# torchmd/torchmd-net

Hardware: AMD Instinct MI355X
Metric: molecules/sec (64-atom molecules) TensorNet E+F (higher is better)
Workload: dtype f32; 1 GPU; BASELINE configs[1]: TensorNet F=128 L=2 K=32 rc=5.0, S-mol64 256 molecules x 64 atoms per GPU, energies + forces, random-init weights (seed 0); atoms_per_gpu=16384, pairs_per_gpu=193709, directed_edges_per_gpu=403802, parallelism=molecule-sharded x1, RCCL all-reduce of energies, rank_step=eager: tmdnet_build_graph (pair-count read-back) + tmdnet_energy_forces

## Files before the change

include/tmdnet_amd.h:

```cpp
#ifndef TMDNET_AMD_H
#define TMDNET_AMD_H

#include <stddef.h>
#include <stdint.h>

#ifdef __cplusplus
extern "C" {
#endif

#define TMDNET_OK 0
#define TMDNET_ERR_INVALID 1
#define TMDNET_ERR_HIP 2
#define TMDNET_ERR_OVERFLOW 3
#define TMDNET_ERR_WORKSPACE 4
#define TMDNET_ERR_STATE 5

typedef struct tmdnet_model tmdnet_model;

typedef struct tmdnet_hparams {
  int32_t hidden_channels;
  int32_t num_layers;
  int32_t num_rbf;
  int32_t max_z;
  int32_t max_num_neighbors;
// ... 127 lines not shown
#define TMDNET_GEMM_ROUTE_SB1_128 6
#define TMDNET_GEMM_ROUTE_SB1_64 7
typedef struct tmdnet_gemm_ex_args {
  const float* A;
  const float* W[TMDNET_GEMM_MAX_GROUPS];
  const float* bias[TMDNET_GEMM_MAX_GROUPS];
  float* C;
  float* pre;
  const float* aux;
  const float* rowscale;
  int64_t lda, ldw, ldc, ldpre, ldaux;
  int32_t a_off[TMDNET_GEMM_MAX_GROUPS], c_off[TMDNET_GEMM_MAX_GROUPS], pre_off[TMDNET_GEMM_MAX_GROUPS],
      aux_off[TMDNET_GEMM_MAX_GROUPS];
  int32_t M, N, K, groups, flags;
  const int32_t* m_dev;
  int32_t m_add;
  const uint16_t* Wsbg[TMDNET_GEMM_MAX_GROUPS];
} tmdnet_gemm_ex_args;
int tmdnet_debug_gemm_ex(void* stream, const tmdnet_gemm_ex_args* args, int32_t* route_out);
int tmdnet_debug_tlin9(void* stream, int32_t pro, int32_t epi, int64_t N, int64_t F, const float* A, const float* A2, float* C,
                       const float* e0, const float* e1, const float* e2, const float* e3, const float* e4, float* o1, float* o2,
                       const float* kap, int32_t want_feat, const float* W_I, const float* W_A, const float* W_S,
                       uint16_t* scratch, int64_t* scratch_elems);
#define TMDNET_MSG_OP_FWD 0
#define TMDNET_MSG_OP_ADJ 1
#define TMDNET_MSG_OP_GD 2
#define TMDNET_MSG_OP_DUAL 3
#define TMDNET_MSG_AUTO 0
#define TMDNET_MSG_FWD_ROW 1
#define TMDNET_MSG_FWD_SPLIT 2
#define TMDNET_MSG_FWD_TILE 3
#define TMDNET_MSG_ADJ_ROW 4
#define TMDNET_MSG_ADJ_SPLIT 5
#define TMDNET_MSG_GD_ROW 6
#define TMDNET_MSG_GD_SPLIT 7
#define TMDNET_MSG_GD_TILE 8
#define TMDNET_MSG_DUAL 9
#define TMDNET_MSG_DUAL_ACC 10
#define TMDNET_MSG_DUAL_SPLIT3 16
typedef struct tmdnet_message_args {
  int32_t op, kernel;
  int32_t N, F, P, small_mols, o3, balance, accumulate;
  const int32_t* rowptr;
  const int32_t* col;
  const int32_t* epair;
  const float* esign;
// ... 136 lines not shown
```

torchmd-net_amd/csrc/tn_api.hip:

```cpp
#include <hip/hip_runtime.h>

#include <algorithm>
#include <cmath>
#include <cstdio>
#include <cstdlib>
#include <cstring>
#include <map>
#include <unordered_map>
#include <string>
#include <vector>

#include "tn_chain.h"
#include "tn_heads.h"
#include "tn_model.h"
#include "tn_tlin9.h"
#include "tn_small.h"
#include "tn_interp.h"
#include "tn_virial.h"

using namespace tn;

static const char* kCatNames[CAT_COUNT] = {"graph", "gemm_edge", "gemm_node", "message", "pair_bwd", "embed_scatter", "elementwise", "edge_table"};

int fail(tmdnet_model* m, int code, const std::string& msg) {
// ... 174 lines not shown
void recall_graph(tmdnet_model* m, const void* graph_ws) {
  auto it = m->graph_rec.find(graph_ws);
  if (it == m->graph_rec.end()) return;
  m->graph_is_cell = it->second.is_cell;
  m->graph_cell_multi = it->second.cell_multi;
  m->graph_has_z = it->second.has_z;
  m->last_nt = it->second.nt;
  m->lastE = it->second.lastE;
  m->graph_no_ghost_pairs = it->second.no_ghost_pairs;
}

bool tlin9_images(const float* const W3[3]) {
  if (!g_cur) return false;
  for (int t = 0; t < 3; ++t)
    if (g_cur->fm_of.find(W3[t]) == g_cur->fm_of.end()) return false;
  return true;
}
void tlin9(hipStream_t s, int pro, int epi, const float* const W3[3], Tl9Args a, double tensors, const char* what) {
  for (int t = 0; t < 3; ++t) a.Wfm[t] = g_cur->fm_of.at(W3[t]);
  char lab[64];
  std::snprintf(lab, sizeof(lab), "tlin9 %s 9x%dx%dx%d", what, a.N, a.F, a.F);
  ProfScope ps_(s, CAT_GEMM_NODE, 2.0 * 9 * a.N * (double)a.F * a.F, 4.0 * (tensors * 9.0 * a.N * a.F + 3.0 * a.F * a.F), lab);
  launch_tlin9(a, pro, epi, s);
}

Graph carve_graph(void* ws, int64_t N, int64_t B, int64_t ecap, size_t* total) {
  Carver c(ws);
  Graph g{};
  const int64_t pcap = ecap / 2 + 1;
  g.small_mols = N <= 96 * (B > 0 ? B : 1) ? 1 : 0;
  g.counts = c.take<int>(8);
  g.mstart = c.take<int>(B);
  g.mend = c.take<int>(B);
  g.nlow = c.take<int>(N);
  g.ntot = c.take<int>(N);
  g.rowptr = c.take<int>(N + 1);
  g.pairptr = c.take<int>(N + 1);
  g.col = c.take<int>(ecap);
  g.epair = c.take<int>(ecap);
  g.esign = c.take<float>(ecap);
  g.pair_i = c.take<int>(pcap);
  g.pair_j = c.take<int>(pcap);
  g.pd = c.take<float>(pcap + 1);
  g.pdelta = c.take<float>(pcap * 3);
  g.prhat = c.take<float>(pcap * 3);
  g.ecap = ecap;
// ... 842 lines not shown
  HIP_TRY(m, hipGetLastError());
  return TMDNET_OK;
}

int tmdnet_set_option(tmdnet_model* m, const char* name, double value) {
  if (!m || !name) return TMDNET_ERR_INVALID;
  const std::string n(name);
  if (n == "edge_table_min_pairs") {
    m->tab_min_pairs = value < 0 ? 0 : (int64_t)value;
    return TMDNET_OK;
  }
  if (n == "embed_rb_min_atoms") {
    m->rb_min_atoms = value < 0 ? 0 : (int64_t)value;
    return TMDNET_OK;
  }
  if (n == "chain_min_atoms") {
    m->chain_min_atoms = value < 0 ? 0 : (value > 9e18 ? INT64_MAX : (int64_t)value);
    return TMDNET_OK;
  }
  if (n == "chain_mask") {
    m->chain_mask = (int)value & 7;
    return TMDNET_OK;
  }
  if (n == "pair_rows_bf16") {
    if (!m->et) return fail(m, TMDNET_ERR_INVALID, "pair_rows_bf16 applies to the Equivariant Transformer handle only");
    m->pair_bf16 = value == 2.0 ? 2 : (value != 0.0 ? 1 : 0);
    return TMDNET_OK;
  }
  if (n == "recompute_pair_rows") {
    if (m->et || m->tn2) return fail(m, TMDNET_ERR_INVALID, "recompute_pair_rows applies to the TensorNet handle only");
    m->recompute_rows = value != 0.0;
    return TMDNET_OK;
  }
  return fail(m, TMDNET_ERR_INVALID, "unknown option: " + n);
}

int tmdnet_get_info(const tmdnet_model* m, const char* name, double* value) {
  if (!m || !name || !value) return TMDNET_ERR_INVALID;
  const std::string n(name);
  if (m->tabs_pending && n.rfind("edge_table_", 0) == 0 && n != "edge_table_min_pairs")
    if (const int rc = ensure_radial_tables(const_cast<tmdnet_model*>(m), nullptr)) return rc;
  if (n == "edge_table_T") *value = m->tabs.ok ? m->tabs.T : 0;
  else if (n == "edge_table_err_value") *value = m->tabs.err_value;
  else if (n == "edge_table_err_slope") *value = m->tabs.err_slope;
  else if (n == "edge_table_min_pairs") *value = (double)m->tab_min_pairs;
  else if (n == "pair_rows_bf16") *value = (double)m->pair_bf16;
  else if (n == "embed_rb_min_atoms") *value = (double)m->rb_min_atoms;
  else if (n == "chain_min_atoms") *value = (double)m->chain_min_atoms;
  else if (n == "chain_mask") *value = (double)m->chain_mask;
  else if (n == "chain_last") *value = (double)m->chain_last;
  else if (n == "recompute_pair_rows") *value = m->recompute_rows ? 1.0 : 0.0;
  else if (n == "embed_rb") *value = m->rb_fwd ? 1.0 : 0.0;
  else if (n == "species_last_build") *value = (double)m->last_nt;
  else if (n == "halo_active_first") *value = (double)m->halo_active[0];
  else if (n == "halo_active_rows") *value = (double)m->halo_active[1];
  else if (n == "message_route_last") *value = (double)m->msg_route_last[0];
  else if (n == "message_adjoint_route_last") *value = (double)m->msg_route_last[1];
  else return TMDNET_ERR_INVALID;
  return TMDNET_OK;
}

int tmdnet_set_cell_grid(tmdnet_model* m, int32_t ncx, int32_t ncy, int32_t ncz) {
  if (!m) return TMDNET_ERR_INVALID;
  if (ncx < 0 || ncy < 0 || ncz < 0) ncx = ncy = ncz = -1;
  m->cell_n[0] = ncx;
  m->cell_n[1] = ncy;
  m->cell_n[2] = ncz;
  return TMDNET_OK;
}

int tmdnet_graph_workspace_bytes(const tmdnet_model* m, int64_t n_atoms, int64_t n_mol, size_t* bytes) {
  if (!m || !bytes || n_atoms < 0 || n_mol < 0) return TMDNET_ERR_INVALID;
  const int64_t ecap = (int64_t)m->hp.max_num_neighbors * n_atoms;
// ... 286 lines not shown
  }
  const bool use_mid = !small_fused_ok(N, F, H, L);
  auto HALO = [&](int stage, float* rows, int row_floats) -> int {
    if (!m->halo_fn) return 0;
    return m->halo_fn(m->halo_user, stage, rows, (int64_t)N, (int64_t)row_floats, perm, (void*)s);
  };
#define HALO_TRY(stage, rows, row_floats) \
  do { if (HALO(stage, rows, row_floats)) return fail(m, TMDNET_ERR_STATE, "halo exchange callback failed at stage " + std::to_string(stage)); } while (0)
  int a0 = 0, Na = N;
  if (m->halo_fn && m->halo_rng && m->atom_w && m->graph_is_cell && want_forces && !tc && (int64_t)N > 256 * (int64_t)B) {
    int h[4] = {0, 0, 0, 0};
    launch_owned_range(m->atom_w, perm, N, m->halo_rng, s);
    HIP_TRY(m, hipMemcpyAsync(h, m->halo_rng, sizeof(h), hipMemcpyDeviceToHost, s));
    HIP_TRY(m, hipStreamSynchronize(s));
    const bool images = tlin9_images(W.Ue) && tlin9_images(W.UeT) && L > 0 && tlin9_images(W.layer[0].V) && tlin9_images(W.layer[0].VT);
    if (h[2] > 0 && h[2] < N && h[1] - h[0] + 1 == h[2] && images && tlin9_ok(h[2], F, true)) {
      a0 = h[0];
      Na = h[2];
    }
  }
  const bool rng = Na != N;
  const bool t9 = !tc && tlin9_ok(Na, F, rng) && tlin9_images(W.Ue) && tlin9_images(W.UeT) && (L == 0 || tlin9_images(W.layer[0].V));
  const bool t9r = !tc && L > 0 && tlin9_ok(Na, F, rng) && tlin9_images(W.UeT) && tlin9_images(W.layer[0].VT);
  m->halo_active[0] = a0;
  m->halo_active[1] = Na;
  const int64_t o1_ = a0, oF = (int64_t)a0 * F, o2F = 2 * oF, o3F = 3 * oF, o9F = 9 * oF, oH = (int64_t)a0 * H;
  const float* const q_a = q ? q + o1_ : nullptr;
  const int64_t* const batch_a = batch_k ? batch_k + o1_ : nullptr;
  const bool fused_small = !tc && !ntp && !recompute && !m->halo_fn && !m->head_kind && (small_fused_ok(N, F, H, L) || mid_fused_ok(N, F, H, L)) &&
                           (!want_forces || (message_adjoint_gd_ok(N, F) && !getenv("TMDNET_SEPARATE_PAIR_GD")));
  auto fm_image = [&](const float* w) -> const uint16_t* {
    auto it = m->fm_of.find(w);
    return it == m->fm_of.end() ? nullptr : it->second;
  };
  const bool chain_any = !tc && !m->head_kind && !m->halo_fn && Na == N && !fused_small && (int64_t)N >= m->chain_min_atoms;
  const bool chain_ro = chain_any && (m->chain_mask & 1) && want_forces && run_fwd && run_bwd && chain_readout_shape_ok(F, H) &&
                        fm_image(W.Lin) && fm_image(W.LinT) && fm_image(W.O1) && fm_image(W.O1T);
  const bool chain_gate = chain_any && want_forces && run_fwd && run_bwd && chain_gate_shape_ok(F);
  const bool chain_gf = chain_gate && (m->chain_mask & 2) && fm_image(W.L1) && fm_image(W.L2);
  const bool chain_gb = chain_gate && (m->chain_mask & 4) && fm_image(W.L2T) && fm_image(W.L1T);
  m->chain_last = (chain_ro ? 1 : 0) | (chain_gf ? 2 : 0) | (chain_gb ? 4 : 0);
  if (run_fwd) {
    if (use_tab) {
      const float* tabs[8];
      float* outs[8];
      float* douts[8];
      int nt_ = 0;
      if (!ntp) {
        tabs[nt_] = m->tabs.tab[0];
        outs[nt_] = b.Q;
        douts[nt_++] = want_forces ? b.dQ : nullptr;
// ... 81 lines not shown
      KR(CAT_SCATTER, momB + Nd * 10 * Fd * 4, launch_embed_combine(g, N, F, K, ntp, z, W.Utab, W.Vtab, m->rb_fwd, b.mom, b.u0, b.s0n, s));
    } else {
      KR(CAT_SCATTER, Pd * 12 * Fd + E_ * 12 + Nd * 10 * Fd * 4,
         launch_embed_scatter(g, N, F, z, W.Utab, W.Vtab, b.Q, b.C, b.u0, b.s0n, s));
    }
    NODE();
    if (chain_gf) {
      ChainGateFwdArgs ca{};
      ca.s0n = b.s0n; ca.xh0 = b.xh0; ca.rstd0 = b.rstd0; ca.a1 = b.a1; ca.a2 = b.a2; ca.gates = b.gates;
      ca.ln_w = W.ln0_w; ca.ln_b = W.ln0_b; ca.bL1 = W.bL1; ca.bL2 = W.bL2; ca.L1_fm = fm_image(W.L1); ca.L2_fm = fm_image(W.L2); ca.N = N;
      char lab[64];
      std::snprintf(lab, sizeof(lab), "chain gate_fwd %dx%d", N, F);
      ProfScope ps_(s, CAT_GEMM_NODE, 2.0 * Nd * 8.0 * Fd * Fd, Nd * 10 * Fd * 4 + Nd * 4 + 4.0 * 8.0 * Fd * Fd, lab);
      if (launch_chain_gate_fwd(ca, F, s)) return fail(m, TMDNET_ERR_HIP, "launch_chain_gate_fwd");
    } else {
    KR(CAT_ELEMENTWISE, Nd * Fd * 12,
       launch_layernorm_fwd(b.s0n + oF, W.ln0_w, W.ln0_b, Na, F, b.ln0 + oF, b.xh0 + oF, b.rstd0 + o1_, s));
    gemm(s, b.ln0 + oF, F, W.L1, F, W.bL1, b.h1 + o2F, 2 * F, Na, 2 * F, F, GEMM_ACT_SILU, b.a1 + o2F, 2 * F);
    gemm(s, b.h1 + o2F, 2 * F, W.L2, 2 * F, W.bL2, b.gates + o3F, 3 * F, Na, 3 * F, 2 * F, GEMM_ACT_SILU, b.a2 + o3F, 3 * F);
    }
    if (t9) {
      Tl9Args ta{};
      ta.A = b.u0 + o9F; ta.C = b.X[0] + o9F; ta.o1 = b.UX + o9F; ta.e3 = b.gates + o3F; ta.N = Na; ta.F = F;
      tlin9(s, TL9_PRO_PLAIN, TL9_EPI_MULGATE, W.Ue, ta, 3.0 + 1.0 / 3.0, "gate");
    } else
      tensor_linear(s, b.u0, W.Ue, b.X[0], N, F, GEMM_MUL_AUX, b.UX, b.gates);
    for (int l = 0; l < L; ++l) {
      const LayerP& q_ = W.layer[l];
      if (es != s) HIP_TRY(m, hipStreamWaitEvent(s, m->ev_join[l], 0));
      float* const Xh_l = tc ? tc->Xh[l] : b.Xh;
      float* const Ch_l = tc ? tc->Ch[l] : b.Ch;
      float* const Xh_n = tc && l + 1 < L ? tc->Xh[l + 1] : b.Xh;
      if (t9) {
        Tl9Args ta{};
        ta.A = b.X[l] + o9F; ta.C = b.Pn[l] + o9F; ta.N = Na; ta.F = F;
        tlin9(s, TL9_PRO_NORM, TL9_EPI_PLAIN, q_.V, ta, 2.0, "norm");
        HALO_TRY(l, b.Pn[l], 9 * F);
        m->msg_route_last[0] = message_route(g, N, F, recompute, a0, rng ? Na : -1);
        KR(CAT_MESSAGE, wB + idxB + nodeB * (1.0 + 2.0 * Na / Nd),
           launch_message(g, N, F, b.w[l], b.Pn[l], q, batch_k, o3, b.Mi[l], Ch_l, s, recompute ? &rts[l] : nullptr, a0, rng ? Na : -1));
        Tl9Args tb{};
        tb.A = Ch_l + o9F; tb.C = b.D[l] + o9F; tb.e0 = b.X[l] + o9F; tb.o1 = b.X[l + 1] + o9F; tb.o2 = b.feat + o3F;
        tb.want_feat = l + 1 == L; tb.kap = q_a;
        tb.N = Na; tb.F = F;
        tlin9(s, TL9_PRO_PLAIN, TL9_EPI_UPDATE, q_.V + 3, tb, 4.0 + (l + 1 == L ? 1.0 / 3.0 : 0.0), "update");
        continue;
      }
      if (l == 0) KR(CAT_ELEMENTWISE, 2 * nodeB, launch_norm_x(b.X[l], Xh_l, N, F, s));
      tensor_linear(s, Xh_l, q_.V, b.Pn[l], N, F);
      HALO_TRY(l, b.Pn[l], 9 * F);
      m->msg_route_last[0] = message_route(g, N, F, recompute);
      KR(CAT_MESSAGE, wB + idxB + 3 * nodeB, launch_message(g, N, F, b.w[l], b.Pn[l], q, batch_k, o3, b.Mi[l], Ch_l, s, recompute ? &rts[l] : nullptr));
      tensor_linear(s, Ch_l, q_.V + 3, b.D[l], N, F);
      KR(CAT_ELEMENTWISE, 4 * nodeB, launch_layer_update(Xh_l, b.D[l], q, batch_k, N, F, b.X[l + 1], l + 1 < L ? 1 : 2,
                                                         l + 1 < L ? Xh_n : b.feat, s));
    }
    if (L == 0) KR(CAT_ELEMENTWISE, nodeB + Nd * 3 * Fd * 4, launch_readout_feat(b.X[L] + o9F, Na, F, b.feat + o3F, s));
    if (chain_ro) {
      ChainReadoutArgs ca{};
      ca.feat = b.feat; ca.X = b.X[L]; ca.G = b.G; ca.x = b.x; ca.ea = b.ea;
      ca.lnr_w = W.lnr_w; ca.lnr_b = W.lnr_b; ca.bLin = W.bLin; ca.bO1 = W.bO1; ca.O2 = W.O2; ca.bO2 = W.bO2;
      ca.Lin_fm = fm_image(W.Lin); ca.LinT_fm = fm_image(W.LinT); ca.O1_fm = fm_image(W.O1); ca.O1T_fm = fm_image(W.O1T);
      ca.atomref = W.atomref; ca.z = z; ca.aw = m->atom_w; ca.perm = perm; ca.std_ = W.std; ca.N = N;
      {
        char lab[64];
        std::snprintf(lab, sizeof(lab), "chain readout_fb %dx%dx%d", N, F, H);
        ProfScope ps_(s, CAT_GEMM_NODE, 2.0 * Nd * (2.0 * 3 * Fd * Fd + 2.0 * Fd * H),
                      2 * nodeB + Nd * 4 * Fd * 4 + Nd * 4 + 4.0 * (2.0 * 3 * Fd * Fd + 2.0 * Fd * H), lab);
// ... 604 lines not shown
  Tl9Args a{};
  for (int t = 0; t < 3; ++t) {
    launch_split_weight_fm(W3[t], F, F, scratch + t * one, s);
    a.Wfm[t] = scratch + t * one;
  }
  a.A = A;
  a.A2 = A2;
  a.C = C;
  a.e0 = e0;
  a.e1 = e1;
  a.e2 = e2;
  a.e3 = e3;
  a.e4 = e4;
  a.o1 = o1;
  a.o2 = o2;
  a.kap = kap;
  a.N = (int)N;
  a.F = (int)F;
  a.want_feat = want_feat ? 1 : 0;
  if (hipGetLastError() != hipSuccess) return TMDNET_ERR_HIP;
  return launch_tlin9(a, pro, epi, s) == (int)hipSuccess ? TMDNET_OK : TMDNET_ERR_HIP;
}

static_assert(TMDNET_MSG_FWD_ROW == MSG_FWD_ROW && TMDNET_MSG_FWD_SPLIT == MSG_FWD_SPLIT && TMDNET_MSG_FWD_TILE == MSG_FWD_TILE &&
                  TMDNET_MSG_ADJ_ROW == MSG_ADJ_ROW && TMDNET_MSG_ADJ_SPLIT == MSG_ADJ_SPLIT && TMDNET_MSG_GD_ROW == MSG_GD_ROW &&
                  TMDNET_MSG_GD_SPLIT == MSG_GD_SPLIT && TMDNET_MSG_GD_TILE == MSG_GD_TILE && TMDNET_MSG_DUAL == MSG_DUAL &&
                  TMDNET_MSG_DUAL_ACC == MSG_DUAL_ACC && TMDNET_MSG_DUAL_SPLIT3 == MSG_DUAL_SPLIT3 && TMDNET_MSG_AUTO == MSG_NONE,
              "route values of the header");

int tmdnet_debug_message(void* stream, const tmdnet_message_args* x, int32_t* route_out, int32_t* slot_arrays_out) {
  if (!x) return TMDNET_ERR_INVALID;
  const int N = x->N, F = x->F;
  if (N < 1 || F < 1 || x->P < 0 || x->op < TMDNET_MSG_OP_FWD || x->op > TMDNET_MSG_OP_DUAL) return TMDNET_ERR_INVALID;
  if (!x->rowptr || !x->col || !x->epair || !x->esign || !x->counts) return TMDNET_ERR_INVALID;
  Graph g{};
  g.rowptr = const_cast<int*>(x->rowptr);
  g.col = const_cast<int*>(x->col);
  g.epair = const_cast<int*>(x->epair);
  g.esign = const_cast<float*>(x->esign);
  g.counts = const_cast<int*>(x->counts);
  g.small_mols = x->small_mols ? 1 : 0;
  MsgRoute r = static_cast<MsgRoute>(x->kernel);
  const bool automatic = x->kernel == TMDNET_MSG_AUTO;
  if (automatic) {
    switch (x->op) {
      case TMDNET_MSG_OP_FWD: r = message_route(g, N, F); break;
// ... 57 lines not shown
```

torchmd-net_amd/csrc/tn_model.h:

```cpp
#pragma once
#include <hip/hip_runtime.h>

#include <cstdio>
#include <cstring>
#include <map>
#include <string>
#include <unordered_map>
#include <vector>

#include "../../include/tmdnet_amd.h"
#include "tn_gemm.h"
#include "tn_kernels.h"
#include "tn_train.h"

using namespace tn;


struct LayerP {
  const float *M1, *b1, *M2, *b2, *M3, *b3;
  const float *M2T, *M3T;
  const float* V[6];
  const float* VT[6];
  const uint16_t* M_sb[3];
};
// ... 151 lines not shown
  std::vector<ParamSpec> specs;
  std::map<std::string, std::vector<float>> host;
  float* dev = nullptr;
  size_t dev_cap = 0, dev_sb_cap = 0, rb_cap = 0;
  uint16_t* dev_sb = nullptr;
  std::unordered_map<const float*, const uint16_t*> sb_of;
  std::unordered_map<const float*, const uint16_t*> fm_of;
  struct ImageJob { size_t src_off; int64_t n, k; size_t dst_off; int fm; };
  std::vector<ImageJob> image_jobs;
  size_t packed_elems = 0;
  int32_t* upd_tid = nullptr;
  int32_t* upd_ofs = nullptr;
  const float** upd_ptrs = nullptr;
  bool upd_ready = false;
  DevParams P;
  EdgeTables tabs;
  uint16_t* rb_img = nullptr;
  const uint16_t *rb_fwd = nullptr, *rb_rev = nullptr;
  int last_nt = 0;
  int64_t rb_min_atoms = 1024;
  int64_t chain_min_atoms = 4096;
  int chain_mask = 7;
  int chain_last = 0;
  int pair_bf16 = 0;
  bool tabs_pending = false;
  int64_t tab_min_pairs = 1;
  bool finalized = false;
  std::string err;
  FwdBuffers last{};
  int64_t lastN = 0, lastP = 0;
  bool has_last = false;
  const float* tn2_last_chg = nullptr;
};


int fail(tmdnet_model* m, int code, const std::string& msg);
#define HIP_TRY(m, expr)                                                                    \
  do {                                                                                      \
    hipError_t e_ = (expr);                                                                 \
    if (e_ != hipSuccess) return fail(m, TMDNET_ERR_HIP, std::string(#expr) + ": " + hipGetErrorString(e_)); \
  } while (0)

struct Packer {
  std::vector<float> buf;
  size_t add(const std::vector<float>& v) {
    size_t off = (buf.size() + 63) & ~size_t(63);
// ... 86 lines not shown
```

torchmd-net_amd/csrc/tn_tlin9.h:

```cpp
#pragma once
#include <hip/hip_runtime.h>
#include <stdint.h>

namespace tn {

enum Tl9Pro : int {
  TL9_PRO_PLAIN = 0,
  TL9_PRO_NORM,
  TL9_PRO_UPDBWD,
};
enum Tl9Epi : int {
  TL9_EPI_PLAIN = 0,
  TL9_EPI_MULGATE,
  TL9_EPI_UPDATE,
  TL9_EPI_NORMBWD,
  TL9_EPI_NORMBWD_GATE,
  TL9_EPI_EMBBWD,
};

struct Tl9Args {
  const float* A;
  const float* A2;
  const uint16_t* Wfm[3];
  float* C;
  const float* e0;
  const float* e1;
  const float* e2;
  const float* e3;
  const float* e4;
  float* o1;
  float* o2;
  const float* kap;
  int N, F, o3, want_feat;
};

bool tlin9_ok(int N, int F, bool any_rounds = false);
size_t split_weight_fm_elems(int64_t n, int64_t k);
void launch_split_weight_fm(const float* W_dev, int64_t n, int64_t k, uint16_t* out_dev, hipStream_t s);
int launch_tlin9(const Tl9Args& a, int pro, int epi, hipStream_t s);

}
```

torchmd-net_amd/csrc/tn_tlin9.hip:

```cpp
#include <cstdlib>

#include "tn_common.h"
#include "tn_gemm_sb.h"
#include "tn_tlin9.h"

namespace tn {

constexpr int T9_RA = 32;
constexpr int T9_PLANE = 9 * T9_RA * 32;
constexpr int T9_STAGE = 3 * T9_PLANE;
constexpr int T9_EG = 8;
constexpr int T9_NT = 128;

typedef float f2v __attribute__((ext_vector_type(2)));
__device__ __forceinline__ f2v ld2(const float* p) { return *reinterpret_cast<const f2v*>(p); }
__device__ __forceinline__ void st2(float* p, f2v v) { *reinterpret_cast<f2v*>(p) = v; }
__device__ __forceinline__ f2v ldu2(const float* ubase, unsigned off) {
  return *reinterpret_cast<const f2v*>(reinterpret_cast<const char*>(ubase) + (size_t)(off * 4u));
}
__device__ __forceinline__ float ldu1(const float* ubase, unsigned off) {
  return *reinterpret_cast<const float*>(reinterpret_cast<const char*>(ubase) + (size_t)(off * 4u));
}
__device__ __forceinline__ void stu2(float* ubase, unsigned off, f2v v) {
  *reinterpret_cast<f2v*>(reinterpret_cast<char*>(ubase) + (size_t)(off * 4u)) = v;
// ... 13 lines not shown
__device__ __forceinline__ void t9_update(const float x[9], const float d[9], float kap, float o[9]) {
  float xh[9];
#pragma unroll
  for (int c = 0; c < 9; ++c) xh[c] = x[c];
  t9_norm(xh);
  const M3 dX = compose(d);
  const M3 Xf = add(add(compose(xh), dX), scale(matmul(dX, dX), kap));
  decompose(Xf, o);
}
__device__ __forceinline__ void t9_norm_bwd(const float u[9], float gx[9] ) {
  float dq[9];
  dquad(u, dq);
  const float inv = 1.0f / (quad(u) + 1.0f);
  float dot = 0.f;
#pragma unroll
  for (int c = 0; c < 9; ++c) dot += gx[c] * u[c];
  const float g_s = -dot * inv * inv;
#pragma unroll
  for (int c = 0; c < 9; ++c) gx[c] = gx[c] * inv + dq[c] * g_s;
}

template <int N_> struct IC { static constexpr int value = N_; };

template <int PRO, int EPI>
__global__ __launch_bounds__(512, 2) void k_tlin9(Tl9Args a, int tiles_m, int tiles_n) {
  __shared__ __attribute__((aligned(16))) unsigned char sA[4 * T9_STAGE];
  float* const sE = reinterpret_cast<float*>(sA + 2 * T9_STAGE);
  const int tid = threadIdx.x, lane = tid & 63, wave = tid >> 6;
  const int wave_u = __builtin_amdgcn_readfirstlane(wave);
  const int wn = wave & 3, wc = wave >> 2;
  const int sa = tid >> 4, skp = tid & 15;
  const int N = a.N, F = a.F, nd = F >> 5, NB = F >> 5;
  const int F9 = 9 * F;
  const int total = tiles_m * tiles_n;
  if ((int)blockIdx.x >= total) return;
  const int my_tiles = (total - 1 - (int)blockIdx.x) / (int)gridDim.x + 1;
  const int ndt = my_tiles * nd;

  auto tile_of = [&](int ts, int& m0, int& n0) __attribute__((always_inline)) {
    const int t = (int)blockIdx.x + ts * (int)gridDim.x;
    const int tn_ = t % tiles_n;
    m0 = (t / tiles_n) * T9_RA;
    n0 = tn_ * T9_NT;
  };

  f2v sr[2][9];
  f2v sr2[2][9];
  float s_kap[2];
  auto load_dbl = [&](auto S_, int dd) __attribute__((always_inline)) {
    constexpr int S = decltype(S_)::value;
    dd = dd < ndt ? dd : ndt - 1;
    const int ts = dd / nd, kd = dd - ts * nd;
    int m0, n0;
    tile_of(ts, m0, n0);
    int n = m0 + sa;
    if (n >= N) n = N - 1;
    if (PRO == TL9_PRO_UPDBWD) s_kap[S] = a.kap ? a.kap[n] : 1.0f;
    const unsigned voff = (unsigned)((n - m0) * F9 + skp * 2);
    const float* p = a.A + (int64_t)m0 * F9 + kd * 32;
#pragma unroll
    for (int c = 0; c < 9; ++c) sr[S][c] = ldu2(p + c * F, voff);
    if (PRO == TL9_PRO_UPDBWD) {
      const float* p2 = a.A2 + (int64_t)m0 * F9 + kd * 32;
// ... 289 lines not shown
    for (int ts = 0; ts < my_tiles; ++ts) {
      int m0n = m0c, n0n = n0c;
      if (ts + 1 < my_tiles) tile_of(ts + 1, m0n, n0n);
#pragma unroll
      for (int ci = 0; ci < 5; ++ci)
#pragma unroll
        for (int e = 0; e < 16; ++e) acc[ci][e] = 0.f;
      for (int kd = 0; kd < nd; kd += 2) {
        dbl(IC<0>{}, ROT_, kd, n0n);
        dbl(IC<1>{}, ROT_, kd + 1, n0n);
      }
      epi_group(IC<0>{}, m0c, n0c);
      epi_group(IC<1>{}, m0c, n0c);
      epi_group(IC<2>{}, m0c, n0c);
      epi_group(IC<3>{}, m0c, n0c);
      m0c = m0n;
      n0c = n0n;
    }
  };
  if (wave < 4) run(IC<0>{});
  else run(IC<1>{});
}

__global__ void k_split_weight_fm(const float* __restrict__ W, int n, int k, uint16_t* __restrict__ out) {
  const int idx = blockIdx.x * blockDim.x + threadIdx.x;
  const int NB = n >> 5, nkc = k >> 4;
  if (idx >= nkc * NB * 64) return;
  const int lane = idx & 63, nb = (idx >> 6) % NB, kc = (idx >> 6) / NB;
  const float* src = W + (int64_t)(nb * 32 + (lane & 31)) * k + kc * 16 + 8 * (lane >> 5);
  const float4 u = *reinterpret_cast<const float4*>(src), v = *reinterpret_cast<const float4*>(src + 4);
  uint4 h, m, l;
  split8(u, v, h, m, l);
  uint16_t* o = out + (((int64_t)kc * NB + nb) * 3) * 512 + lane * 8;
  *reinterpret_cast<uint4*>(o) = h;
  *reinterpret_cast<uint4*>(o + 512) = m;
  *reinterpret_cast<uint4*>(o + 1024) = l;
}
size_t split_weight_fm_elems(int64_t n, int64_t k) { return (size_t)(n * k * 3); }
void launch_split_weight_fm(const float* W_dev, int64_t n, int64_t k, uint16_t* out_dev, hipStream_t s) {
  const int total = (int)((k >> 4) * (n >> 5) * 64);
  hipLaunchKernelGGL(k_split_weight_fm, dim3((total + 255) / 256), dim3(256), 0, s, W_dev, (int)n, (int)k, out_dev);
}

static int t9_num_cu() {
  static const int n_cu = [] {
    int dev = 0, n = 256;
// ... 12 lines not shown
  const int64_t n_cu = t9_num_cu(), rounds = (tiles + n_cu - 1) / n_cu;
  return tiles <= n_cu || 5 * tiles >= 4 * rounds * n_cu;
}

int launch_tlin9(const Tl9Args& a, int pro, int epi, hipStream_t s) {
  const int tiles_m = (a.N + T9_RA - 1) / T9_RA, tiles_n = a.F / T9_NT;
  const int n_cu = t9_num_cu();
  const int total = tiles_m * tiles_n;
  const dim3 grid(total < n_cu ? total : n_cu), block(512);
#define T9_LAUNCH(P, E) hipLaunchKernelGGL((k_tlin9<P, E>), grid, block, 0, s, a, tiles_m, tiles_n)
  if (pro == TL9_PRO_NORM && epi == TL9_EPI_PLAIN) T9_LAUNCH(TL9_PRO_NORM, TL9_EPI_PLAIN);
  else if (pro == TL9_PRO_PLAIN && epi == TL9_EPI_PLAIN) T9_LAUNCH(TL9_PRO_PLAIN, TL9_EPI_PLAIN);
  else if (pro == TL9_PRO_PLAIN && epi == TL9_EPI_MULGATE) T9_LAUNCH(TL9_PRO_PLAIN, TL9_EPI_MULGATE);
  else if (pro == TL9_PRO_PLAIN && epi == TL9_EPI_UPDATE) T9_LAUNCH(TL9_PRO_PLAIN, TL9_EPI_UPDATE);
  else if (pro == TL9_PRO_UPDBWD && epi == TL9_EPI_PLAIN) T9_LAUNCH(TL9_PRO_UPDBWD, TL9_EPI_PLAIN);
  else if (pro == TL9_PRO_PLAIN && epi == TL9_EPI_NORMBWD) T9_LAUNCH(TL9_PRO_PLAIN, TL9_EPI_NORMBWD);
  else if (pro == TL9_PRO_PLAIN && epi == TL9_EPI_NORMBWD_GATE) T9_LAUNCH(TL9_PRO_PLAIN, TL9_EPI_NORMBWD_GATE);
  else if (pro == TL9_PRO_PLAIN && epi == TL9_EPI_EMBBWD) T9_LAUNCH(TL9_PRO_PLAIN, TL9_EPI_EMBBWD);
  else return (int)hipErrorInvalidValue;
#undef T9_LAUNCH
  return (int)hipGetLastError();
}

}
```

torchmd-net_amd/torchmdnet_amd/_C.py:

```python
import ctypes as C
import os
import re

_HERE = os.path.dirname(os.path.abspath(__file__))
LIB_PATH = os.path.join(os.path.dirname(_HERE), "lib", "libtmdnet_amd.so")
HEADER_PATH = os.path.join(os.path.dirname(os.path.dirname(_HERE)), "include", "tmdnet_amd.h")

OK, ERR_INVALID, ERR_HIP, ERR_OVERFLOW, ERR_WORKSPACE, ERR_STATE = 0, 1, 2, 3, 4, 5
HEAD_SCALAR, HEAD_DIPOLE_MOMENT, HEAD_SPATIAL_EXTENT, HEAD_VECTOR = 0, 1, 2, 3


class HParams(C.Structure):
    _fields_ = [
        ("hidden_channels", C.c_int32),
        ("num_layers", C.c_int32),
        ("num_rbf", C.c_int32),
        ("max_z", C.c_int32),
        ("max_num_neighbors", C.c_int32),
        ("group_o3", C.c_int32),
        ("head_hidden", C.c_int32),
        ("has_atomref", C.c_int32),
        ("cutoff_lower", C.c_float),
        ("cutoff_upper", C.c_float),
    ]
# ... 10 lines not shown
                                         "head_hidden", "has_atomref", "q_dim")] + \
               [("cutoff_lower", C.c_float), ("cutoff_upper", C.c_float), ("coulomb_cutoff", C.c_float),
                ("coulomb_epsilon_solvent", C.c_float)]


class GemmExArgs(C.Structure):
    _fields_ = [
        ("A", C.c_void_p), ("W", C.c_void_p * 9), ("bias", C.c_void_p * 9), ("C", C.c_void_p), ("pre", C.c_void_p),
        ("aux", C.c_void_p), ("rowscale", C.c_void_p),
        ("lda", C.c_int64), ("ldw", C.c_int64), ("ldc", C.c_int64), ("ldpre", C.c_int64), ("ldaux", C.c_int64),
        ("a_off", C.c_int32 * 9), ("c_off", C.c_int32 * 9), ("pre_off", C.c_int32 * 9), ("aux_off", C.c_int32 * 9),
        ("M", C.c_int32), ("N", C.c_int32), ("K", C.c_int32), ("groups", C.c_int32), ("flags", C.c_int32),
        ("m_dev", C.c_void_p), ("m_add", C.c_int32),
        ("Wsbg", C.c_void_p * 9),
    ]


class MessageArgs(C.Structure):
    _fields_ = [(n, C.c_int32) for n in ("op", "kernel", "N", "F", "P", "small_mols", "o3", "balance", "accumulate")] + \
               [(n, C.c_void_p) for n in ("rowptr", "col", "epair", "esign", "counts", "w", "w2", "src", "src2", "q", "batch", "out",
                                          "out2", "slots")] + [("slot_stride", C.c_int64)]


MSG_OP_FWD, MSG_OP_ADJ, MSG_OP_GD, MSG_OP_DUAL = range(4)
(MSG_AUTO, MSG_FWD_ROW, MSG_FWD_SPLIT, MSG_FWD_TILE, MSG_ADJ_ROW, MSG_ADJ_SPLIT, MSG_GD_ROW, MSG_GD_SPLIT, MSG_GD_TILE, MSG_DUAL,
 MSG_DUAL_ACC) = range(11)
MSG_DUAL_SPLIT3 = 16
GEMM_ACT_SILU, GEMM_MUL_AUX, GEMM_MUL_DSILU_AUX, GEMM_ACCUM, GEMM_ROWSCALE = 1, 2, 4, 8, 16
(GEMM_ROUTE_NONE, GEMM_ROUTE_SKINNY4, GEMM_ROUTE_SKINNY8, GEMM_ROUTE_TILES_128X128, GEMM_ROUTE_TILES_128X64,
 GEMM_ROUTE_TILES_128X32, GEMM_ROUTE_SB1_128, GEMM_ROUTE_SB1_64) = range(8)
TL9_PRO_PLAIN, TL9_PRO_NORM, TL9_PRO_UPDBWD = 0, 1, 2
TL9_EPI_PLAIN, TL9_EPI_MULGATE, TL9_EPI_UPDATE, TL9_EPI_NORMBWD, TL9_EPI_NORMBWD_GATE, TL9_EPI_EMBBWD = range(6)
VIB_SEED, VIB_PLUS, VIB_MINUS = range(3)
VIB_ANALYTIC, VIB_CENTRAL = range(2)
VIB_PROJECT_NONE, VIB_PROJECT_TRANS, VIB_PROJECT_TRANS_ROT = range(3)
VIB_INFO = 8

_lib = None


def lib():
    global _lib
    if _lib is not None:
        return _lib
    if not os.path.exists(LIB_PATH):
        raise ImportError(
# ... 32 lines not shown
    L.tmdnet_energy_forces.argtypes = [vp, vp, vp, vp, sz, i64, i64, i64, vp, vp, vp, i32, vp, vp]
    L.tmdnet_virial_workspace_bytes.argtypes = [vp, i64, i64, C.POINTER(sz)]
    L.tmdnet_energy_forces_virial.argtypes = [vp, vp, vp, vp, sz, vp, sz, i64, i64, i64, vp, vp, vp, i32, vp, vp, vp]
    L.tmdnet_neighbor_workspace_bytes.argtypes = [i64, i64, i64, C.POINTER(sz)]
    L.tmdnet_neighbor_pairs.argtypes = [vp, vp, sz, i64, i64, vp, vp, vp, i32, f32, f32, i64, i32, i32, i32, vp, vp, vp, vp]
    L.tmdnet_neighbor_grad.argtypes = [vp, vp, vp, vp, vp, vp, i64, i64, vp]
    f64 = C.c_double
    L.tmdnet_neighbor_pairs_f64.argtypes = [vp, vp, sz, i64, i64, vp, vp, vp, i32, f64, f64, i64, i32, i32, vp, vp, vp, vp]
    L.tmdnet_neighbor_grad_f64.argtypes = [vp, vp, vp, vp, vp, vp, i64, i64, vp]
    L.tmdnet_profile_begin.argtypes = [vp, C.c_uint32]
    L.tmdnet_profile_end.argtypes = [vp, vp, C.POINTER(C.c_double), C.POINTER(C.c_double), C.POINTER(C.c_double), C.POINTER(i64)]
    L.tmdnet_profile_end_records.argtypes = [vp, vp, i64, C.POINTER(i32), C.POINTER(C.c_double), C.POINTER(C.c_double),
                                              C.POINTER(C.c_double), C.c_char_p, C.POINTER(i64)]
    L.tmdnet_profile_category_name.argtypes = [C.c_int]
    L.tmdnet_profile_category_name.restype = C.c_char_p
    L.tmdnet_debug_tensor.argtypes = [vp, vp, C.c_char_p, vp, i64]
    L.tmdnet_debug_gemm_dual.argtypes = [vp, vp, vp, vp, vp, vp, vp, i64, i64, i64, i32, vp, vp, vp]
    L.tmdnet_debug_split_weight.argtypes = [vp, i64, i64, vp]
    L.tmdnet_debug_split_weight.restype = i64
    L.tmdnet_debug_gemm.argtypes = [vp, vp, vp, vp, vp, i64, i64, i64, i32, vp]
    L.tmdnet_debug_gemm_ex.argtypes = [vp, C.POINTER(GemmExArgs), C.POINTER(i32)]
    L.tmdnet_debug_tlin9.argtypes = [vp, i32, i32, i64, i64] + [vp] * 11 + [i32, vp, vp, vp, vp, C.POINTER(i64)]
    L.tmdnet_debug_message.argtypes = [vp, C.POINTER(MessageArgs), C.POINTER(i32), C.POINTER(i32)]
    L.tmdnet_param_grad_count.argtypes = [vp]
    L.tmdnet_param_grad_entry.argtypes = [vp, C.c_int, C.POINTER(i64), C.POINTER(i64)]
    L.tmdnet_param_grad_entry.restype = C.c_char_p
    L.tmdnet_train_workspace_bytes.argtypes = [vp, i64, i64, i64, C.POINTER(sz), C.POINTER(sz), C.POINTER(i64)]
    L.tmdnet_energy_param_grads.argtypes = [vp, vp, vp, vp, sz, vp, sz, i64, i64, i64, vp, vp, vp, vp, vp, vp]
    L.tmdnet_force_param_workspace_bytes.argtypes = [vp, i64, i64, i64, C.POINTER(sz)]
    L.tmdnet_force_param_grads.argtypes = [vp, vp, vp, vp, sz, i64, i64, i64, vp, vp, vp, vp, vp, vp]
    L.tmdnet_loss_param_grads.argtypes = [vp, vp, vp, vp, sz, i64, i64, i64, vp, vp, vp, vp, vp, vp, vp]
    L.tmdnet_hvp_debug_tensor.argtypes = [vp, vp, C.c_char_p, vp, i64]
    L.tmdnet_set_output_head.argtypes = [vp, i32]
    u64 = C.c_uint64
    L.tmdnet_md_workspace_bytes.argtypes = [i64, i64, C.POINTER(sz)]
    L.tmdnet_md_reset.argtypes = [vp, vp, u64]
    L.tmdnet_md_advance.argtypes = [vp, vp, vp, vp, i64, i64, i32, vp, vp, vp, vp, vp, vp, vp, f32, f32, f32, u64, vp, vp, vp, vp]
    L.tmdnet_md_status.argtypes = [vp, vp, C.POINTER(u64)]
    L.tmdnet_md_barostat_workspace_bytes.argtypes = [i64, C.POINTER(sz)]
    L.tmdnet_md_barostat.argtypes = [vp, vp, vp, vp, vp, i64, i64, i32, vp, vp, vp, vp, f32, vp, vp, i32, vp, vp, f64, f64, f64, f64, f64,
                                     u64, vp, vp, vp]
    L.tmdnet_md_exchange_workspace_bytes.argtypes = [i64, i32, C.POINTER(sz)]
    L.tmdnet_md_exchange.argtypes = [vp, vp, vp, vp, vp, i64, i64, i32, i64, vp, vp, vp, vp, vp, vp, vp, u64, vp, vp, vp, vp, vp]
    L.tmdnet_md_bias_workspace_bytes.argtypes = [i64, i32, i32, i32, i64, C.POINTER(sz)]
    L.tmdnet_md_bias_reset.argtypes = [vp, vp, u64, u64]
    L.tmdnet_md_bias.argtypes = [vp, vp, vp, vp, vp, i64, i64, i32, vp, vp, i32, vp, vp, vp, i32, vp, vp, vp, vp, vp, vp, i32, i32, i32,
# ... 47 lines not shown
```

Baseline: 106,600 molecules/s.

## Fuse consecutive tlin9 stages (gate+norm, update+norm) into one persistent kernel

Adds a sequenced tlin9 kernel that runs two dependent tensor-linear stages back to back inside one launch. Each block owns the same row tiles across both stages, so the second stage consumes rows that block just produced, with only a block barrier between them. It is used for gate followed by layer-0 norm, and for update followed by the next layer's norm, and is enabled by default when F equals the tile width. This removes a kernel launch and keeps tiles warm in cache, but it requires each block to own full row tiles (tiles_n=1) and adds debug API surface.

```diff
diff --git a/include/tmdnet_amd.h b/include/tmdnet_amd.h
--- a/include/tmdnet_amd.h
+++ b/include/tmdnet_amd.h
@@ -173,6 +173,21 @@
                        const float* e0, const float* e1, const float* e2, const float* e3, const float* e4, float* o1, float* o2,
                        const float* kap, int32_t want_feat, const float* W_I, const float* W_A, const float* W_S,
                        uint16_t* scratch, int64_t* scratch_elems);
+#define TMDNET_TL9_SEQ_GATE_NORM 0
+#define TMDNET_TL9_SEQ_UPDATE_NORM 1
+typedef struct tmdnet_tlin9_stage {
+  const float *A, *e0, *e3;
+  float *C, *o1, *o2;
+  const float* W[3];
+} tmdnet_tlin9_stage;
+typedef struct tmdnet_tlin9_seq_args {
+  int32_t seq, fused, N, F, want_feat, reserved;
+  tmdnet_tlin9_stage st[2];
+  const float* kap;
+  uint16_t* scratch;
+  int64_t scratch_elems;
+} tmdnet_tlin9_seq_args;
+int tmdnet_debug_tlin9_seq(void* stream, const tmdnet_tlin9_seq_args* args);
 #define TMDNET_MSG_OP_FWD 0
 #define TMDNET_MSG_OP_ADJ 1
 #define TMDNET_MSG_OP_GD 2
diff --git a/torchmd-net_amd/csrc/tn_api.hip b/torchmd-net_amd/csrc/tn_api.hip
--- a/torchmd-net_amd/csrc/tn_api.hip
+++ b/torchmd-net_amd/csrc/tn_api.hip
@@ -220,6 +220,15 @@
   std::snprintf(lab, sizeof(lab), "tlin9 %s 9x%dx%dx%d", what, a.N, a.F, a.F);
   ProfScope ps_(s, CAT_GEMM_NODE, 2.0 * 9 * a.N * (double)a.F * a.F, 4.0 * (tensors * 9.0 * a.N * a.F + 3.0 * a.F * a.F), lab);
   launch_tlin9(a, pro, epi, s);
+}
+void tlin9_seq(hipStream_t s, int seq, const float* const* const W3[2], Tl9SeqArgs q, double tensors, const char* what) {
+  for (int i = 0; i < 2; ++i)
+    for (int t = 0; t < 3; ++t) q.st[i].Wfm[t] = g_cur->fm_of.at(W3[i][t]);
+  const Tl9Args& a = q.st[0];
+  char lab[64];
+  std::snprintf(lab, sizeof(lab), "tlin9 %s 9x%dx%dx%d", what, a.N, a.F, a.F);
+  ProfScope ps_(s, CAT_GEMM_NODE, 2 * 2.0 * 9 * a.N * (double)a.F * a.F, 4.0 * (tensors * 9.0 * a.N * a.F + 2 * 3.0 * a.F * a.F), lab);
+  launch_tlin9_seq(q, seq, s);
 }
 
 Graph carve_graph(void* ws, int64_t N, int64_t B, int64_t ecap, size_t* total) {
@@ -1108,6 +1117,10 @@
     m->chain_mask = (int)value & 7;
     return TMDNET_OK;
   }
+  if (n == "tlin9_seq_mask") {
+    m->tlin9_seq_mask = (int)value & ((1 << TL9_SEQ_COUNT) - 1);
+    return TMDNET_OK;
+  }
   if (n == "pair_rows_bf16") {
     if (!m->et) return fail(m, TMDNET_ERR_INVALID, "pair_rows_bf16 applies to the Equivariant Transformer handle only");
     m->pair_bf16 = value == 2.0 ? 2 : (value != 0.0 ? 1 : 0);
@@ -1135,6 +1148,8 @@
   else if (n == "chain_min_atoms") *value = (double)m->chain_min_atoms;
   else if (n == "chain_mask") *value = (double)m->chain_mask;
   else if (n == "chain_last") *value = (double)m->chain_last;
+  else if (n == "tlin9_seq_mask") *value = (double)m->tlin9_seq_mask;
+  else if (n == "tlin9_seq_last") *value = (double)m->tlin9_seq_last;
   else if (n == "recompute_pair_rows") *value = m->recompute_rows ? 1.0 : 0.0;
   else if (n == "embed_rb") *value = m->rb_fwd ? 1.0 : 0.0;
   else if (n == "species_last_build") *value = (double)m->last_nt;
@@ -1467,11 +1482,19 @@
   const bool rng = Na != N;
   const bool t9 = !tc && tlin9_ok(Na, F, rng) && tlin9_images(W.Ue) && tlin9_images(W.UeT) && (L == 0 || tlin9_images(W.layer[0].V));
   const bool t9r = !tc && L > 0 && tlin9_ok(Na, F, rng) && tlin9_images(W.UeT) && tlin9_images(W.layer[0].VT);
+  const int sq_mask = tlin9_seq_ok(F) && !rng ? m->tlin9_seq_mask : 0;
+  const bool sq_gate_norm = t9 && L > 0 && (sq_mask & 1), sq_update_norm = t9 && L > 1 && (sq_mask & 2);
+  m->tlin9_seq_last = (sq_gate_norm && run_fwd ? 1 : 0) | (sq_update_norm && run_fwd ? 2 : 0);
   m->halo_active[0] = a0;
   m->halo_active[1] = Na;
   const int64_t o1_ = a0, oF = (int64_t)a0 * F, o2F = 2 * oF, o3F = 3 * oF, o9F = 9 * oF, oH = (int64_t)a0 * H;
   const float* const q_a = q ? q + o1_ : nullptr;
   const int64_t* const batch_a = batch_k ? batch_k + o1_ : nullptr;
+  auto norm_args = [&](int l) {
+    Tl9Args ta{};
+    ta.A = b.X[l] + o9F; ta.C = b.Pn[l] + o9F; ta.N = Na; ta.F = F;
+    return ta;
+  };
   const bool fused_small = !tc && !ntp && !recompute && !m->halo_fn && !m->head_kind && (small_fused_ok(N, F, H, L) || mid_fused_ok(N, F, H, L)) &&
                            (!want_forces || (message_adjoint_gd_ok(N, F) && !getenv("TMDNET_SEPARATE_PAIR_GD")));
   auto fm_image = [&](const float* w) -> const uint16_t* {
@@ -1599,7 +1622,14 @@
     if (t9) {
       Tl9Args ta{};
       ta.A = b.u0 + o9F; ta.C = b.X[0] + o9F; ta.o1 = b.UX + o9F; ta.e3 = b.gates + o3F; ta.N = Na; ta.F = F;
-      tlin9(s, TL9_PRO_PLAIN, TL9_EPI_MULGATE, W.Ue, ta, 3.0 + 1.0 / 3.0, "gate");
+      if (sq_gate_norm) {
+        Tl9SeqArgs sq{};
+        sq.st[0] = ta;
+        sq.st[1] = norm_args(0);
+        const float* const* const ws[2] = {W.Ue, W.layer[0].V};
+        tlin9_seq(s, TL9_SEQ_GATE_NORM, ws, sq, 4.0 + 1.0 / 3.0, "gate+norm");
+      } else
+        tlin9(s, TL9_PRO_PLAIN, TL9_EPI_MULGATE, W.Ue, ta, 3.0 + 1.0 / 3.0, "gate");
     } else
       tensor_linear(s, b.u0, W.Ue, b.X[0], N, F, GEMM_MUL_AUX, b.UX, b.gates);
     for (int l = 0; l < L; ++l) {
@@ -1609,9 +1639,7 @@
       float* const Ch_l = tc ? tc->Ch[l] : b.Ch;
       float* const Xh_n = tc && l + 1 < L ? tc->Xh[l + 1] : b.Xh;
       if (t9) {
-        Tl9Args ta{};
-        ta.A = b.X[l] + o9F; ta.C = b.Pn[l] + o9F; ta.N = Na; ta.F = F;
-        tlin9(s, TL9_PRO_NORM, TL9_EPI_PLAIN, q_.V, ta, 2.0, "norm");
+        if (!(l == 0 ? sq_gate_norm : sq_update_norm)) tlin9(s, TL9_PRO_NORM, TL9_EPI_PLAIN, q_.V, norm_args(l), 2.0, "norm");
         HALO_TRY(l, b.Pn[l], 9 * F);
         m->msg_route_last[0] = message_route(g, N, F, recompute, a0, rng ? Na : -1);
         KR(CAT_MESSAGE, wB + idxB + nodeB * (1.0 + 2.0 * Na / Nd),
@@ -1620,7 +1648,14 @@
         tb.A = Ch_l + o9F; tb.C = b.D[l] + o9F; tb.e0 = b.X[l] + o9F; tb.o1 = b.X[l + 1] + o9F; tb.o2 = b.feat + o3F;
         tb.want_feat = l + 1 == L; tb.kap = q_a;
         tb.N = Na; tb.F = F;
-        tlin9(s, TL9_PRO_PLAIN, TL9_EPI_UPDATE, q_.V + 3, tb, 4.0 + (l + 1 == L ? 1.0 / 3.0 : 0.0), "update");
+        if (sq_update_norm && l + 1 < L) {
+          Tl9SeqArgs sq{};
+          sq.st[0] = tb;
+          sq.st[1] = norm_args(l + 1);
+          const float* const* const ws[2] = {q_.V + 3, W.layer[l + 1].V};
+          tlin9_seq(s, TL9_SEQ_UPDATE_NORM, ws, sq, 5.0, "update+norm");
+        } else
+          tlin9(s, TL9_PRO_PLAIN, TL9_EPI_UPDATE, q_.V + 3, tb, 4.0 + (l + 1 == L ? 1.0 / 3.0 : 0.0), "update");
         continue;
       }
       if (l == 0) KR(CAT_ELEMENTWISE, 2 * nodeB, launch_norm_x(b.X[l], Xh_l, N, F, s));
@@ -2271,6 +2306,45 @@
   return launch_tlin9(a, pro, epi, s) == (int)hipSuccess ? TMDNET_OK : TMDNET_ERR_HIP;
 }
 
+static_assert(TMDNET_TL9_SEQ_GATE_NORM == TL9_SEQ_GATE_NORM && TMDNET_TL9_SEQ_UPDATE_NORM == TL9_SEQ_UPDATE_NORM,
+              "sequence values of the header");
+
+int tmdnet_debug_tlin9_seq(void* stream, const tmdnet_tlin9_seq_args* x) {
+  if (!x || x->seq < 0 || x->seq >= TL9_SEQ_COUNT) return TMDNET_ERR_INVALID;
+  const int64_t N = x->N, F = x->F;
+  if (F < 128 || F % 128 || N < 1 || N > (1 << 26)) return TMDNET_ERR_INVALID;
+  if (x->fused && !tlin9_seq_ok((int)F)) return TMDNET_ERR_INVALID;
+  const int64_t one = (int64_t)split_weight_fm_elems(F, F);
+  const int pro[2] = {TL9_PRO_PLAIN, TL9_PRO_NORM};
+  const int epi[2] = {x->seq == TL9_SEQ_GATE_NORM ? TL9_EPI_MULGATE : TL9_EPI_UPDATE, TL9_EPI_PLAIN};
+  auto bad = [](const void* p, uintptr_t al) { return !p || (reinterpret_cast<uintptr_t>(p) & (al - 1)); };
+  bool inv = bad(x->scratch, 16) || x->scratch_elems < 2 * 3 * one || (x->kap && bad(x->kap, 4));
+  Tl9SeqArgs q{};
+  hipStream_t s = reinterpret_cast<hipStream_t>(stream);
+  for (int i = 0; i < 2 && !inv; ++i) {
+    const auto& t = x->st[i];
+    Tl9Args& a = q.st[i];
+    a.A = t.A; a.C = t.C; a.e0 = t.e0; a.e3 = t.e3; a.o1 = t.o1; a.o2 = t.o2;
+    a.kap = x->kap; a.N = (int)N; a.F = (int)F;
+    a.want_feat = epi[i] == TL9_EPI_UPDATE && x->want_feat ? 1 : 0;
+    inv = bad(a.A, 8) || bad(a.C, 8) || bad(t.W[0], 16) || bad(t.W[1], 16) || bad(t.W[2], 16);
+    if (epi[i] == TL9_EPI_MULGATE) inv = inv || bad(a.e3, 8) || bad(a.o1, 8);
+    if (epi[i] == TL9_EPI_UPDATE) inv = inv || bad(a.e0, 8) || bad(a.o1, 8) || (a.want_feat && bad(a.o2, 8));
+  }
+  if (inv) return TMDNET_ERR_INVALID;
+  for (int i = 0; i < 2; ++i)
+    for (int t = 0; t < 3; ++t) {
+      uint16_t* img = x->scratch + (3 * i + t) * one;
+      launch_split_weight_fm(x->st[i].W[t], F, F, img, s);
+      q.st[i].Wfm[t] = img;
+    }
+  if (hipGetLastError() != hipSuccess) return TMDNET_ERR_HIP;
+  if (x->fused) return launch_tlin9_seq(q, x->seq, s) == (int)hipSuccess ? TMDNET_OK : TMDNET_ERR_HIP;
+  for (int i = 0; i < 2; ++i)
+    if (launch_tlin9(q.st[i], pro[i], epi[i], s) != (int)hipSuccess) return TMDNET_ERR_HIP;
+  return TMDNET_OK;
+}
+
 static_assert(TMDNET_MSG_FWD_ROW == MSG_FWD_ROW && TMDNET_MSG_FWD_SPLIT == MSG_FWD_SPLIT && TMDNET_MSG_FWD_TILE == MSG_FWD_TILE &&
                   TMDNET_MSG_ADJ_ROW == MSG_ADJ_ROW && TMDNET_MSG_ADJ_SPLIT == MSG_ADJ_SPLIT && TMDNET_MSG_GD_ROW == MSG_GD_ROW &&
                   TMDNET_MSG_GD_SPLIT == MSG_GD_SPLIT && TMDNET_MSG_GD_TILE == MSG_GD_TILE && TMDNET_MSG_DUAL == MSG_DUAL &&
diff --git a/torchmd-net_amd/csrc/tn_model.h b/torchmd-net_amd/csrc/tn_model.h
--- a/torchmd-net_amd/csrc/tn_model.h
+++ b/torchmd-net_amd/csrc/tn_model.h
@@ -197,6 +197,8 @@
   int64_t chain_min_atoms = 4096;
   int chain_mask = 7;
   int chain_last = 0;
+  int tlin9_seq_mask = 3;
+  int tlin9_seq_last = 0;
   int pair_bf16 = 0;
   bool tabs_pending = false;
   int64_t tab_min_pairs = 1;
diff --git a/torchmd-net_amd/csrc/tn_tlin9.h b/torchmd-net_amd/csrc/tn_tlin9.h
--- a/torchmd-net_amd/csrc/tn_tlin9.h
+++ b/torchmd-net_amd/csrc/tn_tlin9.h
@@ -34,7 +34,18 @@
   int N, F, o3, want_feat;
 };
 
+enum Tl9Seq : int {
+  TL9_SEQ_GATE_NORM = 0,
+  TL9_SEQ_UPDATE_NORM,
+  TL9_SEQ_COUNT
+};
+struct Tl9SeqArgs {
+  Tl9Args st[2];
+};
+
 bool tlin9_ok(int N, int F, bool any_rounds = false);
+bool tlin9_seq_ok(int F);
+int launch_tlin9_seq(const Tl9SeqArgs& q, int seq, hipStream_t s);
 size_t split_weight_fm_elems(int64_t n, int64_t k);
 void launch_split_weight_fm(const float* W_dev, int64_t n, int64_t k, uint16_t* out_dev, hipStream_t s);
 int launch_tlin9(const Tl9Args& a, int pro, int epi, hipStream_t s);
diff --git a/torchmd-net_amd/csrc/tn_tlin9.hip b/torchmd-net_amd/csrc/tn_tlin9.hip
--- a/torchmd-net_amd/csrc/tn_tlin9.hip
+++ b/torchmd-net_amd/csrc/tn_tlin9.hip
@@ -59,9 +59,9 @@
 
 template <int N_> struct IC { static constexpr int value = N_; };
 
+
 template <int PRO, int EPI>
-__global__ __launch_bounds__(512, 2) void k_tlin9(Tl9Args a, int tiles_m, int tiles_n) {
-  __shared__ __attribute__((aligned(16))) unsigned char sA[4 * T9_STAGE];
+__device__ __forceinline__ void t9_stage(const Tl9Args& a, unsigned char* const sA, int tiles_n, int ts0, int ts1) {
   float* const sE = reinterpret_cast<float*>(sA + 2 * T9_STAGE);
   const int tid = threadIdx.x, lane = tid & 63, wave = tid >> 6;
   const int wave_u = __builtin_amdgcn_readfirstlane(wave);
@@ -69,13 +69,12 @@
   const int sa = tid >> 4, skp = tid & 15;
   const int N = a.N, F = a.F, nd = F >> 5, NB = F >> 5;
   const int F9 = 9 * F;
-  const int total = tiles_m * tiles_n;
-  if ((int)blockIdx.x >= total) return;
-  const int my_tiles = (total - 1 - (int)blockIdx.x) / (int)gridDim.x + 1;
+  const int my_tiles = ts1 - ts0;
+  if (my_tiles <= 0) return;
   const int ndt = my_tiles * nd;
 
   auto tile_of = [&](int ts, int& m0, int& n0) __attribute__((always_inline)) {
-    const int t = (int)blockIdx.x + ts * (int)gridDim.x;
+    const int t = (int)blockIdx.x + (ts0 + ts) * (int)gridDim.x;
     const int tn_ = t % tiles_n;
     m0 = (t / tiles_n) * T9_RA;
     n0 = tn_ * T9_NT;
@@ -411,6 +410,32 @@
   else run(IC<1>{});
 }
 
+__device__ __forceinline__ int t9_my_tiles(int total) { return (total - 1 - (int)blockIdx.x) / (int)gridDim.x + 1; }
+
+template <int PRO, int EPI>
+__global__ __launch_bounds__(512, 2) void k_tlin9(Tl9Args a, int tiles_m, int tiles_n) {
+  __shared__ __attribute__((aligned(16))) unsigned char sA[4 * T9_STAGE];
+  const int total = tiles_m * tiles_n;
+  if ((int)blockIdx.x >= total) return;
+  t9_stage<PRO, EPI>(a, sA, tiles_n, 0, t9_my_tiles(total));
+}
+
+template <int SEQ>
+__global__ __launch_bounds__(512, 2) void k_tlin9_seq(Tl9SeqArgs q, int tiles_m) {
+  __shared__ __attribute__((aligned(16))) unsigned char sA[4 * T9_STAGE];
+  if ((int)blockIdx.x >= tiles_m) return;
+  const int my_tiles = t9_my_tiles(tiles_m);
+  if (SEQ == TL9_SEQ_GATE_NORM) {
+    t9_stage<TL9_PRO_PLAIN, TL9_EPI_MULGATE>(q.st[0], sA, 1, 0, my_tiles);
+    __syncthreads();
+    t9_stage<TL9_PRO_NORM, TL9_EPI_PLAIN>(q.st[1], sA, 1, 0, my_tiles);
+  } else {
+    t9_stage<TL9_PRO_PLAIN, TL9_EPI_UPDATE>(q.st[0], sA, 1, 0, my_tiles);
+    __syncthreads();
+    t9_stage<TL9_PRO_NORM, TL9_EPI_PLAIN>(q.st[1], sA, 1, 0, my_tiles);
+  }
+}
+
 __global__ void k_split_weight_fm(const float* __restrict__ W, int n, int k, uint16_t* __restrict__ out) {
   const int idx = blockIdx.x * blockDim.x + threadIdx.x;
   const int NB = n >> 5, nkc = k >> 4;
@@ -469,4 +494,19 @@
   return (int)hipGetLastError();
 }
 
-}
+bool tlin9_seq_ok(int F) { return F == T9_NT; }
+int launch_tlin9_seq(const Tl9SeqArgs& q, int seq, hipStream_t s) {
+  const int N = q.st[0].N;
+  if (!tlin9_seq_ok(q.st[0].F) || N < 1) return (int)hipErrorInvalidValue;
+  const int tiles_m = (N + T9_RA - 1) / T9_RA;
+  const int n_cu = t9_num_cu();
+  const dim3 grid(tiles_m < n_cu ? tiles_m : n_cu), block(512);
+#define T9_LAUNCH(S) hipLaunchKernelGGL((k_tlin9_seq<S>), grid, block, 0, s, q, tiles_m)
+  if (seq == TL9_SEQ_GATE_NORM) T9_LAUNCH(TL9_SEQ_GATE_NORM);
+  else if (seq == TL9_SEQ_UPDATE_NORM) T9_LAUNCH(TL9_SEQ_UPDATE_NORM);
+  else return (int)hipErrorInvalidValue;
+#undef T9_LAUNCH
+  return (int)hipGetLastError();
+}
+
+}
diff --git a/torchmd-net_amd/torchmdnet_amd/_C.py b/torchmd-net_amd/torchmdnet_amd/_C.py
--- a/torchmd-net_amd/torchmdnet_amd/_C.py
+++ b/torchmd-net_amd/torchmdnet_amd/_C.py
@@ -56,6 +56,16 @@
                                           "out2", "slots")] + [("slot_stride", C.c_int64)]
 
 
+class Tlin9Stage(C.Structure):
+    _fields_ = [(n, C.c_void_p) for n in ("A", "e0", "e3", "C", "o1", "o2")] + [("W", C.c_void_p * 3)]
+
+
+class Tlin9SeqArgs(C.Structure):
+    _fields_ = [(n, C.c_int32) for n in ("seq", "fused", "N", "F", "want_feat", "reserved")] + [("st", Tlin9Stage * 2)] + \
+               [(n, C.c_void_p) for n in ("kap", "scratch")] + [("scratch_elems", C.c_int64)]
+
+
+TL9_SEQ_GATE_NORM, TL9_SEQ_UPDATE_NORM = range(2)
 MSG_OP_FWD, MSG_OP_ADJ, MSG_OP_GD, MSG_OP_DUAL = range(4)
 (MSG_AUTO, MSG_FWD_ROW, MSG_FWD_SPLIT, MSG_FWD_TILE, MSG_ADJ_ROW, MSG_ADJ_SPLIT, MSG_GD_ROW, MSG_GD_SPLIT, MSG_GD_TILE, MSG_DUAL,
  MSG_DUAL_ACC) = range(11)
@@ -134,6 +144,7 @@
     L.tmdnet_debug_gemm_ex.argtypes = [vp, C.POINTER(GemmExArgs), C.POINTER(i32)]
     L.tmdnet_debug_tlin9.argtypes = [vp, i32, i32, i64, i64] + [vp] * 11 + [i32, vp, vp, vp, vp, C.POINTER(i64)]
     L.tmdnet_debug_message.argtypes = [vp, C.POINTER(MessageArgs), C.POINTER(i32), C.POINTER(i32)]
+    L.tmdnet_debug_tlin9_seq.argtypes = [vp, C.POINTER(Tlin9SeqArgs)]
     L.tmdnet_param_grad_count.argtypes = [vp]
     L.tmdnet_param_grad_entry.argtypes = [vp, C.c_int, C.POINTER(i64), C.POINTER(i64)]
     L.tmdnet_param_grad_entry.restype = C.c_char_p
```

New measurement: 107,500 molecules/s, median of 6. About the same (+0.9%).
